# smearle/control-pcgrl

Hardware: AMD Instinct MI355X
Metric: env-steps/sec at N envs/GPU (binary 16x16), 1/2/4/8 MI355X (higher is better)
Workload: dtype u8

## Files before the change

### control_pcgrl_amd/_lib.py

```python
import ctypes as C
import os
import subprocess

_HERE = os.path.dirname(os.path.abspath(__file__))
CSRC = os.path.join(_HERE, "csrc")
LIB_PATH = os.path.join(CSRC, "libpcgrl_amd.so")
UNITS = ["pcgrl_engine.hip", "pcgrl_k_binary32.hip", "pcgrl_k_binary64.hip", "pcgrl_k_zelda32.hip", "pcgrl_k_zelda64.hip",
         "pcgrl_k_sokoban32_8.hip", "pcgrl_k_sokoban32_16.hip", "pcgrl_k_sokoban32_32.hip",
         "pcgrl_k_sokoban32_64.hip", "pcgrl_k_sokoban64_32.hip", "pcgrl_k_sokoban64_64.hip", "pcgrl_k_3d.hip",
         "codes/pcgrl_codes.hip", "reps3d/pcgrl_k_3d_turtle.hip", "reps3d/pcgrl_k_3d_wide.hip",
         "async3d/pcgrl_k_3d_async.hip", "paths/pcgrl_k_paths_binary.hip", "paths/pcgrl_k_paths_zelda.hip",
         "solutions/pcgrl_k_solutions.hip", "multiagent/pcgrl_k_ma_binary.hip", "multiagent/pcgrl_k_ma_zelda.hip",
         "measures/pcgrl_k_measures.hip", "smb/pcgrl_k_smb.hip", "smb/pcgrl_k_smb_env.hip", "smb/pcgrl_k_smb_ready.hip",
         "smb/pcgrl_k_smb_state.hip", "smb/pcgrl_k_smb_rollout.hip", "smb/pcgrl_k_smb_vector.hip",
         "smb/pcgrl_k_smb_measures.hip", "loderunner/pcgrl_k_loderunner.hip",
         "loderunner/pcgrl_k_loderunner_measures.hip", "loderunner/pcgrl_k_loderunner_routes.hip",
         "microstructure/pcgrl_k_microstructure.hip", "ddave/pcgrl_k_ddave.hip",
         "mdungeon/pcgrl_k_mdungeon.hip"]
HEADERS = ["pcgrl_kernels2d.h", "pcgrl_kernels3d.h", "pcgrl_sokoban.h", "pcgrl_common.h", "pcgrl_dispatch.h", "codes/pcgrl_codes.h",
           "reps3d/pcgrl_reps3d.h", "async3d/pcgrl_async3d.h", "paths/pcgrl_paths.h",
           "solutions/pcgrl_solutions.h", "multiagent/pcgrl_multiagent.h", "measures/pcgrl_measures.h",
           "smb/pcgrl_smb.h", "smb/pcgrl_smb_env.h", "smb/pcgrl_smb_ready.h", "smb/pcgrl_smb_state.h",
           "smb/pcgrl_smb_rollout.h", "smb/pcgrl_smb_ctrl.h", "smb/pcgrl_smb_vector.h", "smb/pcgrl_smb_measures.h",
           "loderunner/pcgrl_loderunner.h", "measures/pcgrl_measures_wave.h", "loderunner/pcgrl_loderunner_measures.h",
           "loderunner/pcgrl_loderunner_routes.h", "microstructure/pcgrl_microstructure.h", "ddave/pcgrl_ddave.h",
           "mdungeon/pcgrl_mdungeon.h"]
SOURCES = UNITS + HEADERS
HEADER = os.path.join(os.path.dirname(_HERE), "include", "pcgrl_amd.h")
CODES_HEADER = os.path.join(os.path.dirname(_HERE), "include", "pcgrl_amd_codes.h")
ASYNC3D_HEADER = os.path.join(os.path.dirname(_HERE), "include", "pcgrl_amd_async3d.h")
PATHS_HEADER = os.path.join(os.path.dirname(_HERE), "include", "pcgrl_amd_paths.h")
SOLUTIONS_HEADER = os.path.join(os.path.dirname(_HERE), "include", "pcgrl_amd_solutions.h")
MULTIAGENT_HEADER = os.path.join(os.path.dirname(_HERE), "include", "pcgrl_amd_multiagent.h")
MEASURES_HEADER = os.path.join(os.path.dirname(_HERE), "include", "pcgrl_amd_measures.h")
SMB_HEADER = os.path.join(os.path.dirname(_HERE), "include", "pcgrl_amd_smb.h")
SMB_ENV_HEADER = os.path.join(os.path.dirname(_HERE), "include", "pcgrl_amd_smb_env.h")
SMB_READY_HEADER = os.path.join(os.path.dirname(_HERE), "include", "pcgrl_amd_smb_ready.h")
SMB_STATE_HEADER = os.path.join(os.path.dirname(_HERE), "include", "pcgrl_amd_smb_state.h")
SMB_ROLLOUT_HEADER = os.path.join(os.path.dirname(_HERE), "include", "pcgrl_amd_smb_rollout.h")
SMB_CTRL_HEADER = os.path.join(os.path.dirname(_HERE), "include", "pcgrl_amd_smb_ctrl.h")
SMB_VECTOR_HEADER = os.path.join(os.path.dirname(_HERE), "include", "pcgrl_amd_smb_vector.h")
SMB_MEASURES_HEADER = os.path.join(os.path.dirname(_HERE), "include", "pcgrl_amd_smb_measures.h")
LODERUNNER_HEADER = os.path.join(os.path.dirname(_HERE), "include", "pcgrl_amd_loderunner.h")
LODERUNNER_MEASURES_HEADER = os.path.join(os.path.dirname(_HERE), "include", "pcgrl_amd_loderunner_measures.h")
LODERUNNER_ROUTES_HEADER = os.path.join(os.path.dirname(_HERE), "include", "pcgrl_amd_loderunner_routes.h")
MICROSTRUCTURE_HEADER = os.path.join(os.path.dirname(_HERE), "include", "pcgrl_amd_microstructure.h")
DDAVE_HEADER = os.path.join(os.path.dirname(_HERE), "include", "pcgrl_amd_ddave.h")
MDUNGEON_HEADER = os.path.join(os.path.dirname(_HERE), "include", "pcgrl_amd_mdungeon.h")
HIPCC_FLAGS = ["--offload-arch=gfx950", "-O3", "-std=c++17", "-ffp-contract=off", "-falign-loops=32", "-fPIC"]

PCGRL_MAX_STATS = 8
ERRORS = {1: "EINVAL", 2: "EUNSUPPORTED", 3: "EHIP", 4: "EACTION", 5: "ESTALE"}


class PcgrlConfig(C.Structure):
    _fields_ = [
        ("problem", C.c_int32), ("representation", C.c_int32), ("ndim", C.c_int32),
        ("dims", C.c_int32 * 3), ("obs_window", C.c_int32 * 3),
        ("max_iterations", C.c_int32), ("max_changes", C.c_int32), ("n_stats", C.c_int32),
        ("has_trg", C.c_int32 * PCGRL_MAX_STATS), ("weights", C.c_double * PCGRL_MAX_STATS),
        ("trg_lo", C.c_double * PCGRL_MAX_STATS), ("trg_hi", C.c_double * PCGRL_MAX_STATS),
        ("solver_power", C.c_int32),
        ("n_ctrl", C.c_int32), ("ctrl_idx", C.c_int32 * PCGRL_MAX_STATS), ("ctrl_range", C.c_double * PCGRL_MAX_STATS),
        ("act_window", C.c_int32 * 3), ("static_tiles", C.c_int32), ("n_static_walls", C.c_int32),
        ("static_eval", C.c_int32), ("static_prob", C.c_double),
    ]


SYMBOLS = {
    "pcgrl_create": (C.c_int, [C.POINTER(PcgrlConfig), C.c_int32, C.c_int32, C.POINTER(C.c_void_p)]),
    "pcgrl_destroy": (None, [C.c_void_p]),
    "pcgrl_seed": (C.c_int, [C.c_void_p, C.c_void_p]),
    "pcgrl_reset": (C.c_int, [C.c_void_p, C.c_void_p, C.c_void_p, C.c_void_p, C.c_void_p]),
    "pcgrl_step_seq": (C.c_int, [C.c_void_p, C.c_void_p, C.c_int64, C.c_int32, C.c_int32, C.c_int32, C.c_int32, C.c_void_p,
                                 C.c_void_p, C.c_void_p, C.c_void_p, C.c_void_p]),
    "pcgrl_step": (C.c_int, [C.c_void_p, C.c_void_p, C.c_int32, C.c_void_p, C.c_void_p, C.c_void_p, C.c_void_p,
                             C.c_void_p]),
    "pcgrl_step_ex": (C.c_int, [C.c_void_p, C.c_void_p, C.c_int32, C.c_void_p, C.c_void_p, C.c_void_p, C.c_void_p,
                                C.c_void_p, C.c_void_p, C.c_void_p]),
# ... 368 lines not shown
```

### control_pcgrl_amd/csrc/pcgrl_engine.hip

```cpp
#include <hip/hip_runtime.h>

#include <algorithm>
#include <cmath>
#include <cstddef>
#include <cstdio>
#include <cstring>
#include <string>
#include <vector>

#include <map>
#include <mutex>
#include <tuple>

#include "pcgrl_common.h"
#include "pcgrl_dispatch.h"
#include "pcgrl_kernels2d.h"
#include "pcgrl_sokoban.h"
#include "pcgrl_kernels3d.h"
#include "codes/pcgrl_codes.h"
#include "reps3d/pcgrl_reps3d.h"
#include "async3d/pcgrl_async3d.h"
#include "paths/pcgrl_paths.h"
#include "solutions/pcgrl_solutions.h"
#include "multiagent/pcgrl_multiagent.h"
#include "measures/pcgrl_measures.h"
#include "smb/pcgrl_smb.h"
#include "../../include/pcgrl_amd_codes.h"
#include "../../include/pcgrl_amd_async3d.h"
#include "../../include/pcgrl_amd_paths.h"
#include "../../include/pcgrl_amd_solutions.h"
#include "../../include/pcgrl_amd_multiagent.h"
#include "../../include/pcgrl_amd_measures.h"
#include "../../include/pcgrl_amd_smb.h"
#include "../../include/pcgrl_amd_smb_env.h"
#include "smb/pcgrl_smb_env.h"
#include "../../include/pcgrl_amd_smb_ready.h"
#include "smb/pcgrl_smb_ready.h"
#include "../../include/pcgrl_amd_smb_state.h"
#include "smb/pcgrl_smb_state.h"
#include "../../include/pcgrl_amd_smb_rollout.h"
#include "smb/pcgrl_smb_rollout.h"
#include "../../include/pcgrl_amd_smb_ctrl.h"
#include "smb/pcgrl_smb_ctrl.h"
#include "../../include/pcgrl_amd_smb_vector.h"
#include "smb/pcgrl_smb_vector.h"
#include "../../include/pcgrl_amd_smb_measures.h"
#include "smb/pcgrl_smb_measures.h"
#include "../../include/pcgrl_amd_loderunner.h"
#include "loderunner/pcgrl_loderunner.h"
#include "../../include/pcgrl_amd_loderunner_routes.h"
#include "loderunner/pcgrl_loderunner_routes.h"
#include "../../include/pcgrl_amd_loderunner_measures.h"
#include "loderunner/pcgrl_loderunner_measures.h"
#include "../../include/pcgrl_amd_microstructure.h"
#include "microstructure/pcgrl_microstructure.h"
#include "../../include/pcgrl_amd_ddave.h"
#include "ddave/pcgrl_ddave.h"
#include "../../include/pcgrl_amd_mdungeon.h"
#include "mdungeon/pcgrl_mdungeon.h"

using namespace pcgrl;

static thread_local std::string g_err;
static int fail(int code, const std::string &msg) {
  g_err = msg;
  return code;
}
#define HIPCHK(x)                                                                                   \
  do {                                                                                              \
    hipError_t _e = (x);                                                                            \
    if (_e != hipSuccess) return fail(PCGRL_EHIP, std::string(#x) + ": " + hipGetErrorString(_e)); \
  } while (0)

namespace pcgrl {
struct RedScratch;
struct SampleState;
}
struct pcgrl_engine {
  Params p;
  int device = 0;
  int lpe = 16;
  size_t lds_bytes = 0;
  int cpl = 0;
  int32_t *seen_host = nullptr;
  int soko_slots = 0;
  int32_t seen_last = 0, spread_left = 0;
  bool soko_lazy = true;
  int sk_budget = 0;
  void *a3_park = nullptr;
  void *sk_ws = nullptr, *sk_park = nullptr;
  bool soko_grow_failed = false;
  std::string soko_grow_msg;
  uint8_t *hdr_host = nullptr;
  int rollout_form = -1;
  int rollout_epw = -1;
  bool split_ok = false;
  int64_t two_role_resident = 0;
  hipStream_t side = nullptr;
  hipEvent_t ev_fork = nullptr, ev_join = nullptr;
  void *snap_planes = nullptr;
  EnvState *snap_st = nullptr;
  RngState *snap_rng = nullptr;
  long obs_nt_mb = 384;
  bool maybe_stale = false;
  int64_t obs_bytes = 0;
  int obs_ndim = 0;
  int32_t obs_shape[4] = {0, 0, 0, 0};
  RedScratch *red = nullptr;
  SampleState *sample = nullptr;
  bool ma_on = false;
  MaArgs ma = {};
  size_t ma_lds = 0;
  int64_t ma_obs_bytes = 0;
  int32_t ma_obs_shape[3] = {0, 0, 0};
  std::vector<void *> allocs;
  std::vector<std::pair<void *, size_t>> state_arrays;
};

extern "C" {
static void state_header_build(pcgrl_engine *h);
}

static void seedseq_words(uint64_t seed, uint64_t out[4]) {
  const uint32_t INIT_A = 0x43b0d7e5u, MULT_A = 0x931e8875u, INIT_B = 0x8b51f9ddu, MULT_B = 0x58f38dedu;
  const uint32_t MIX_L = 0xca01f9ddu, MIX_R = 0x4973f715u;
  uint32_t ent[4] = {(uint32_t)seed, (uint32_t)(seed >> 32), 0, 0};
  int n_ent = ent[1] ? 2 : 1;
  uint32_t pool[4], hc = INIT_A;
  auto hashmix = [&](uint32_t v) {
    v ^= hc;
    hc *= MULT_A;
    v *= hc;
    v ^= v >> 16;
    return v;
  };
  for (int i = 0; i < 4; i++) pool[i] = hashmix(i < n_ent ? ent[i] : 0u);
  for (int s = 0; s < 4; s++)
    for (int d = 0; d < 4; d++)
      if (s != d) {
        uint32_t r = MIX_L * pool[d] - MIX_R * hashmix(pool[s]);
        r ^= r >> 16;
        pool[d] = r;
      }
  uint32_t w[8], hb = INIT_B;
  for (int i = 0; i < 8; i++) {
    uint32_t v = pool[i & 3] ^ hb;
    hb *= MULT_B;
// ... 104 lines not shown
    return fail(PCGRL_EUNSUPPORTED, "sokoban: solver_power must be in [1, " + std::to_string(SK_MAX_POWER) +
                                        "] (the device solver's visited table and node ids are sized for that)");
  lpe = H <= 8 ? 8 : (H <= 16 ? 16 : (H <= 32 ? 32 : 64));
  if (W > 32 && lpe < 32) lpe = 32;
  if (c.representation == PCGRL_REP_WIDE) {
    if (c.obs_window[0] != H || c.obs_window[1] != W)
      return fail(PCGRL_EINVAL, "wide representation needs obs_window == map_shape (reference wrappers.py:140-150 reshape)");
    if (H != W) return fail(PCGRL_EUNSUPPORTED, "wide representation: the reference's transposed write needs a square map");
    obs_chunks = (W * nt + 15) / 16;
    obs_bytes = (int64_t)H * W * nt;
    shape[0] = H;
    shape[1] = W;
    shape[2] = nt;
    ndim = 3;
  } else {
    const int OH = c.obs_window[0], OW = c.obs_window[1], C = nt + 1 + (c.static_tiles ? 1 : 0);
    if (OH < 1 || OW < 1) return fail(PCGRL_EINVAL, "obs_window must be positive");
    obs_chunks = (OW * C + 15) / 16;
    obs_bytes = (int64_t)OH * OW * C;
    shape[0] = OH;
    shape[1] = OW;
    shape[2] = C;
    ndim = 3;
  }
  return PCGRL_OK;
}

static std::vector<JumpEntry> make_jump_table(int H, int W, int last = -1) {
  std::vector<JumpEntry> t(H + 1);
  U128 A{0, 1}, G{0, 0};
  const U128 a{PCG_MULT_HI, PCG_MULT_LO};
  int k = 0;
  for (int r = 0; r <= H; r++) {
    const int want = (r == H && last >= 0) ? last : r * W;
    if (want < k) {
      A = U128{0, 1};
      G = U128{0, 0};
      k = 0;
    }
    while (k < want) {
      G = add128(mul128(G, a), U128{0, 1});
      A = mul128(A, a);
      k++;
    }
    t[r] = JumpEntry{A.hi, A.lo, G.hi, G.lo};
  }
  return t;
}

static bool obs_nt_for(const pcgrl_engine *e, int64_t bytes_per_launch) {
  return e->obs_nt_mb > 0 && bytes_per_launch >= (int64_t)e->obs_nt_mb * 1000000;
}

static hipError_t launch(KernelId id, int lpe, const Params &p, size_t lds, hipStream_t s, int cpl = 0) {
  const bool wide64 = p.cfg.dims[1] > 32;
  switch (p.cfg.problem) {
    case PCGRL_PROB_MC3DMAZE:
      if (p.cfg.representation == PCGRL_REP_TURTLE) return launch_3d_turtle(id, p, cpl, s);
      if (p.cfg.representation == PCGRL_REP_WIDE) return launch_3d_wide(id, p, cpl, s);
      if (p.sk_budget > 0 && (id == K_STEP || id == K_RESET)) return launch_3d_async(id, p, cpl, s);
      return launch_3d(id, p, cpl, s);
    case PCGRL_PROB_BINARY: return wide64 ? launch_binary64(id, lpe, p, lds, s) : launch_binary32(id, lpe, p, lds, s);
    case PCGRL_PROB_ZELDA: return wide64 ? launch_zelda64(id, lpe, p, lds, s) : launch_zelda32(id, lpe, p, lds, s);
    default: return wide64 ? launch_sokoban64(id, lpe, p, lds, s) : launch_sokoban32(id, lpe, p, lds, s);
  }
}

struct DeviceGuard {
  int prev = -1;
  hipError_t err;
  explicit DeviceGuard(int device) {
    err = hipGetDevice(&prev);
    if (err == hipSuccess && prev != device) err = hipSetDevice(device);
    else if (err == hipSuccess) prev = -1;
  }
  ~DeviceGuard() {
    if (prev >= 0) (void)hipSetDevice(prev);
  }
};
#define ON_DEVICE(dev)                                                                            \
  DeviceGuard _guard(dev);                                                                        \
  if (_guard.err != hipSuccess) return fail(PCGRL_EHIP, std::string("hipSetDevice: ") + hipGetErrorString(_guard.err))

namespace pcgrl {

__global__ __launch_bounds__(64) void queue_targets_kernel(Params p, const double *lo, const double *hi) {
  const int env = blockIdx.x * 64 + threadIdx.x;
  if (env >= p.n_envs || (p.mask != nullptr && p.mask[env] == 0)) return;
  double *q = p.trg_pending + (size_t)env * PCGRL_MAX_STATS * 2;
  for (int k = 0; k < p.cfg.n_stats; k++) {
    q[2 * k] = lo[(size_t)env * p.cfg.n_stats + k];
    q[2 * k + 1] = hi[(size_t)env * p.cfg.n_stats + k];
  }
  p.trg_flag[env] |= 1;
}

constexpr int RED_BLOCKS = 64, RED_THREADS = 256, RED_W = 3 + PCGRL_MAX_STATS;
struct RedScratch {
  double part[RED_BLOCKS][RED_W];
  unsigned int ticket;
};
__global__ __launch_bounds__(RED_THREADS) void reduce_episodes_kernel(Params p, RedScratch *scr, double *out, int n_blocks, int clear) {
  __shared__ double sh[RED_THREADS / 64][RED_W];
  __shared__ bool last;
  const int chunk = (p.n_envs + n_blocks - 1) / n_blocks;
  const int lo = blockIdx.x * chunk, hi = min(p.n_envs, lo + chunk);
  double ret = 0.0;
  int64_t v[RED_W - 1];
// ... 193 lines not shown
  }
  (void)hipGetLastError();
  h->soko_grow_failed = true;
  h->soko_grow_msg = std::string("solver pool: growing from ") + std::to_string(h->soko_slots) + " to " + std::to_string(want) +
                     " slots failed: " + hipGetErrorString(e);
  return lazy ? PCGRL_OK : fail(PCGRL_EHIP, h->soko_grow_msg);
}

static void soko_pool_lazy(pcgrl_engine *h, Params &p, hipStream_t stream) {
  if (!h->seen_host || h->soko_slots >= sokoban_slots_for(h->p.n_envs)) return;
  if (*(volatile int32_t *)h->seen_host != 0) soko_pool_for(h, p, sokoban_slots_for(h->p.n_envs), stream);
}

static void choose_spread(pcgrl_engine *h, Params &p) {
  if (!h->seen_host || h->p.ext) return;
  static const int force = getenv("PCGRL_FORCE_SPREAD") ? atoi(getenv("PCGRL_FORCE_SPREAD")) : 0;
  if (force) {
    p.spread = 1;
    p.sk_helpers = force == 2 ? 3 : 0;
    return;
  }
  if (h->p.n_envs > 8192) return;
  const int32_t seen = *(volatile int32_t *)h->seen_host;
  if (seen != h->seen_last) {
    h->seen_last = seen;
    h->spread_left = 16;
  }
  if (h->spread_left > 0) {
    h->spread_left--;
    p.spread = 1;
    p.sk_helpers = h->lds_bytes + 3 * (size_t)SK_HELPER_LDS + 4096 <= 160 * 1024 ? 3 : 0;
  }
}

extern "C" {

const char *pcgrl_last_error(void) { return g_err.c_str(); }
const char *pcgrl_version(void) { return "pcgrl_amd 0.7.0 (gfx950)"; }

int pcgrl_create(const pcgrl_config *cfg, int32_t n_envs, int32_t device, pcgrl_handle *out) {
  if (!cfg || !out || n_envs < 1) return fail(PCGRL_EINVAL, "pcgrl_create: bad arguments");
  int lpe = 16, obs_chunks = 0, ndim = 0;
  int64_t obs_bytes = 0;
  int32_t shape[4] = {0, 0, 0, 0};
  int rc = validate(*cfg, lpe, obs_bytes, obs_chunks, shape, ndim);
  if (rc) return rc;
  ON_DEVICE(device);
  pcgrl_engine *e = new pcgrl_engine();
  {
    const char *f = getenv("PCGRL_ROLLOUT_KERNEL");
    if (f != nullptr && (f[0] == '0' || f[0] == '1')) e->rollout_form = f[0] - '0';
    if (getenv("PCGRL_OBS_NT_MB")) e->obs_nt_mb = atol(getenv("PCGRL_OBS_NT_MB"));
    if (getenv("PCGRL_ROLLOUT_EPW")) e->rollout_epw = atoi(getenv("PCGRL_ROLLOUT_EPW"));
  }
  e->device = device;
  e->lpe = lpe;
  e->obs_bytes = obs_bytes;
  e->obs_ndim = ndim;
  memcpy(e->obs_shape, shape, sizeof(shape));
  Params &p = e->p;
  memset(&p, 0, sizeof(p));
  p.cfg = *cfg;
  {
    bool integral = true;
    for (int k = 0; k < PCGRL_MAX_STATS; k++) {
      const double lo = cfg->trg_lo[k], hi = cfg->trg_hi[k];
      const int32_t big = 1 << 29;
      int32_t lo_i = 0, hi_i = 0;
      if (k < cfg->n_stats && cfg->has_trg[k]) {
        if (lo != lo || hi != hi || lo > hi) integral = false;
        else {
          if (lo <= -(double)big) lo_i = -big;
          else if (lo >= (double)big) lo_i = big;
          else if (lo == (double)(int32_t)lo) lo_i = (int32_t)lo;
          else integral = false;
          if (hi >= (double)big) hi_i = big;
          else if (hi <= -(double)big) hi_i = -big;
          else if (hi == (double)(int32_t)hi) hi_i = (int32_t)hi;
          else integral = false;
        }
      }
      p.trg_lo_i[k] = lo_i;
      p.trg_hi_i[k] = hi_i;
    }
    p.int_targets = integral ? 1 : 0;
  }
  p.n_envs = n_envs;
  p.n_tiles = n_tiles_of(cfg->problem);
  const bool is3d = cfg->problem == PCGRL_PROB_MC3DMAZE;
  p.n_cells = cfg->dims[0] * cfg->dims[1] * (is3d ? cfg->dims[2] : 1);
  p.obs_chunks = obs_chunks;
  if (is3d) m3_edge_masks_host(cfg->dims[1], cfg->dims[2], p.m3_notx0, p.m3_notxl);
  p.ext = (!is3d && (cfg->static_tiles || cfg->act_window[0] > 0)) ? 1 : 0;
  p.n_act = (!is3d && cfg->act_window[0] > 0) ? cfg->act_window[0] * cfg->act_window[1] : 1;
  e->lds_bytes = (size_t)(obs_chunks * 16 + 32) * (65 + (cfg->static_tiles ? 16 : 0)) + 64 * 8;
  {
    const int Hc = cfg->dims[0], Wc = cfg->dims[1], OWc = cfg->obs_window[1], Cc = p.n_tiles + 1;
    const bool fast_cfg = Hc == 16 && Wc == 16 && cfg->obs_window[0] == 32 && OWc == 32;
    p.obs16 = (!is3d && fast_cfg) ? 1 : 0;
    if ((p.obs16 || is3d) && obs_nt_for(e, (int64_t)n_envs * obs_bytes)) p.obs16 |= 2;
    if (!is3d && cfg->representation != PCGRL_REP_WIDE && !cfg->static_tiles && !fast_cfg && (OWc * Cc) % 16 == 0 &&
        e->lds_bytes > 20000) {
      const int rs = (Wc + 8 + 12 + 15) & ~15;
      const int epw = 64 / lpe;
      p.obs_codes = rs;
      e->lds_bytes = (size_t)epw * Hc * rs + rs + (size_t)Cc * 48 + 64 * 8;
// ... 144 lines not shown
  if (h->ma_on) HIPCHK(hipMemset2D(h->ma.side + 1, 4 * sizeof(uint32_t), 0, 2 * sizeof(uint32_t), (size_t)h->p.n_envs));
  return PCGRL_OK;
}

static void with_budget(const pcgrl_engine *h, Params &p) {
  p.sk_budget = h->sk_budget;
  if (h->sk_budget > 0 && h->a3_park) p.soko = h->a3_park;
}
static bool async_capable(const pcgrl_engine *h) {
  return h->p.soko != nullptr || (h->p.cfg.problem == PCGRL_PROB_MC3DMAZE && h->p.cfg.representation == PCGRL_REP_NARROW);
}

#define NOT_ATTACHED(h, what)                                                                                             \
  if ((h)->ma_on)                                                                                                         \
  return fail(PCGRL_EINVAL, std::string(what) + ": the engine steps several agents (pcgrl_ma_attach): use the pcgrl_ma_* entry " \
                                                "points of pcgrl_amd_multiagent.h")

int pcgrl_reset(pcgrl_handle h, const uint8_t *d_mask, const uint8_t *d_init_grids, const int32_t *d_init_pos, void *stream) {
  if (!h) return fail(PCGRL_EINVAL, "pcgrl_reset: null handle");
  NOT_ATTACHED(h, "pcgrl_reset");
  ON_DEVICE(h->device);
  Params p = h->p;
  soko_pool_lazy(h, p, (hipStream_t)stream);
  p.mask = d_mask;
  p.init_grids = d_init_grids;
  p.init_pos = d_init_pos;
  with_budget(h, p);
  HIPCHK(launch(K_RESET, h->lpe, p, h->lds_bytes, (hipStream_t)stream, h->cpl));
  if (d_mask == nullptr) h->maybe_stale = false;
  return PCGRL_OK;
}

#define NOT_WITH_BUDGET(h, what)                                                                                         \
  if ((h)->sk_budget > 0)                                                                                                \
  return fail(PCGRL_EINVAL, std::string(what) + ": a solver budget is set (pcgrl_set_solver_budget): envs may be busy, which only " \
                                                "pcgrl_step_ready can report")

int pcgrl_step(pcgrl_handle h, const int32_t *d_actions, int32_t auto_reset, uint8_t *d_obs, float *d_reward, uint8_t *d_done,
               int32_t *d_stats, void *stream) {
  if (!h || !d_actions) return fail(PCGRL_EINVAL, "pcgrl_step: bad arguments");
  NOT_WITH_BUDGET(h, "pcgrl_step");
  NOT_ATTACHED(h, "pcgrl_step");
  ON_DEVICE(h->device);
  Params p = h->p;
  p.no_fast = h->maybe_stale ? 1 : 0;
  soko_pool_lazy(h, p, (hipStream_t)stream);
  choose_spread(h, p);
  p.actions = d_actions;
  p.auto_reset = auto_reset;
  p.obs = d_obs;
  p.reward = d_reward;
  p.done = d_done;
  p.stats_out = d_stats;
  HIPCHK(launch(K_STEP, h->lpe, p, h->lds_bytes, (hipStream_t)stream, h->cpl));
  return PCGRL_OK;
}

int pcgrl_step_seq(pcgrl_handle h, const int32_t *d_action_rows, int64_t row_stride, int32_t n_rows, int32_t first_row,
                   int32_t n_steps, int32_t auto_reset, uint8_t *d_obs, float *d_reward, uint8_t *d_done, int32_t *d_stats,
                   void *stream) {
  if (!h || !d_action_rows || n_rows < 1 || n_steps < 0 || first_row < 0 || row_stride < 0)
    return fail(PCGRL_EINVAL, "pcgrl_step_seq: bad arguments");
  for (int32_t k = 0; k < n_steps; k++) {
    const int rc = pcgrl_step(h, d_action_rows + (size_t)((first_row + k) % n_rows) * (size_t)row_stride, auto_reset, d_obs, d_reward,
                              d_done, d_stats, stream);
    if (rc != PCGRL_OK) return rc;
  }
  return PCGRL_OK;
}

int pcgrl_step_ex(pcgrl_handle h, const int32_t *d_actions, int32_t auto_reset, uint8_t *d_obs, float *d_reward,
                  double *d_reward64, uint8_t *d_done, int32_t *d_stats, float *d_ctrl_obs, void *stream) {
  if (!h || !d_actions) return fail(PCGRL_EINVAL, "pcgrl_step_ex: bad arguments");
  NOT_WITH_BUDGET(h, "pcgrl_step_ex");
  NOT_ATTACHED(h, "pcgrl_step_ex");
  ON_DEVICE(h->device);
  if (d_ctrl_obs && h->p.cfg.n_ctrl == 0) return fail(PCGRL_EINVAL, "pcgrl_step_ex: d_ctrl_obs needs cfg.n_ctrl > 0");
  Params p = h->p;
  p.no_fast = h->maybe_stale ? 1 : 0;
  soko_pool_lazy(h, p, (hipStream_t)stream);
  choose_spread(h, p);
  p.actions = d_actions;
  p.auto_reset = auto_reset;
  p.obs = d_obs;
  p.reward = d_reward;
  p.reward64 = d_reward64;
  p.done = d_done;
  p.stats_out = d_stats;
  p.ctrl_obs = d_ctrl_obs;
  HIPCHK(launch(K_STEP, h->lpe, p, h->lds_bytes, (hipStream_t)stream, h->cpl));
  return PCGRL_OK;
}

static bool rollout_as_steps(const pcgrl_engine *h) {
  if (h->rollout_form >= 0) return h->rollout_form == 0;
  return h->p.cfg.problem != PCGRL_PROB_MC3DMAZE && (h->p.obs_codes > 0 || h->lpe > 16);
}

int32_t pcgrl_rollout_is_one_launch(pcgrl_handle h) { return h ? (rollout_as_steps(h) ? 0 : 1) : -1; }

int pcgrl_set_rollout_form(pcgrl_handle h, int32_t form) {
  if (!h || form < -1 || form > 2)
    return fail(PCGRL_EINVAL, "pcgrl_set_rollout_form: form must be -1 (by shape), 0 (step launches), 1 (one kernel) or 2 (two kernels)");
  if (form == 2 && !h->split_ok)
    return fail(PCGRL_EUNSUPPORTED, "pcgrl_set_rollout_form(2): the two-kernel rollout exists for 16 x 16 maps with the default window, plain mode");
  h->rollout_form = form;
  return PCGRL_OK;
}

int pcgrl_rollout_ex(pcgrl_handle h, const int32_t *d_actions, int32_t n_steps, int32_t auto_reset, uint8_t *d_obs,
                     int32_t obs_last_only, float *d_reward, double *d_reward64, uint8_t *d_done, int32_t *d_stats, float *d_ctrl_obs,
                     void *stream) {
  if (!h || !d_actions || n_steps < 1) return fail(PCGRL_EINVAL, "pcgrl_rollout: bad arguments");
  NOT_WITH_BUDGET(h, "pcgrl_rollout");
  NOT_ATTACHED(h, "pcgrl_rollout");
  if (d_ctrl_obs && h->p.cfg.n_ctrl == 0) return fail(PCGRL_EINVAL, "pcgrl_rollout_ex: d_ctrl_obs needs cfg.n_ctrl > 0");
  if (rollout_as_steps(h)) {
    const size_t N = (size_t)h->p.n_envs;
    for (int32_t k = 0; k < n_steps; k++) {
      const bool last = k == n_steps - 1;
      uint8_t *obs_k = d_obs == nullptr ? nullptr : (obs_last_only ? (last ? d_obs : nullptr) : d_obs + (size_t)k * N * (size_t)h->obs_bytes);
      const int rc = pcgrl_step_ex(h, d_actions + (size_t)k * N * (size_t)h->p.n_act, auto_reset, obs_k, d_reward ? d_reward + (size_t)k * N : nullptr,
                                   d_reward64 ? d_reward64 + (size_t)k * N : nullptr, d_done ? d_done + (size_t)k * N : nullptr,
                                   d_stats ? d_stats + (size_t)k * N * (size_t)h->p.cfg.n_stats : nullptr, last ? d_ctrl_obs : nullptr, stream);
      if (rc != PCGRL_OK) return rc;
    }
    return PCGRL_OK;
  }
  ON_DEVICE(h->device);
  Params p = h->p;
  p.no_fast = h->maybe_stale ? 1 : 0;
  soko_pool_lazy(h, p, (hipStream_t)stream);
  p.actions = d_actions;
  p.n_steps = n_steps;
  p.spread = 0;
  const bool roles_ok = h->split_ok && !h->maybe_stale && d_reward64 == nullptr && d_ctrl_obs == nullptr && h->rollout_form != 1;
  const int64_t two_role_wgs = ((int64_t)h->p.n_envs + 64 / h->lpe - 1) / (64 / h->lpe);
  const bool in_rounds = h->two_role_resident > 0 && two_role_wgs > h->two_role_resident;
  const bool split = roles_ok && d_obs != nullptr && (h->rollout_form == 2 || (in_rounds && !obs_last_only && n_steps >= 16));
  const bool sim_then_observe = roles_ok && !split && d_obs != nullptr && obs_last_only && in_rounds;
  const bool sim_only = (roles_ok && d_obs == nullptr) || sim_then_observe;
  if (h->p.cfg.problem != PCGRL_PROB_MC3DMAZE) {
    const int full = 64 / h->lpe;
// ... 15 lines not shown
    hipStream_t s0 = (hipStream_t)stream;
    if (split) {
      const int64_t plane_q = (int64_t)h->p.n_envs * ROW_WORDS * h->p.cfg.dims[0] * (int64_t)sizeof(uint32_t) / 16;
      const int64_t total = plane_q + (int64_t)h->p.n_envs * 2 + (int64_t)h->p.n_envs * (int64_t)(sizeof(RngState) / 16);
      hipLaunchKernelGGL(rollout_snapshot_kernel, dim3((unsigned)((total + 255) / 256)), dim3(256), 0, s0, (const uint4 *)h->p.planes,
                         (uint4 *)h->snap_planes, plane_q, (const uint4 *)h->p.st, (uint4 *)h->snap_st, (const uint4 *)h->p.rng, (uint4 *)h->snap_rng,
                         h->p.n_envs);
      HIPCHK(hipGetLastError());
      HIPCHK(hipEventRecord(h->ev_fork, s0));
      HIPCHK(hipStreamWaitEvent(h->side, h->ev_fork, 0));
      Params po = p;
      po.planes = h->snap_planes;
      po.st = h->snap_st;
      po.rng = h->snap_rng;
      po.spread = 0;
      po.reward = nullptr;
      po.done = nullptr;
      po.stats_out = nullptr;
      HIPCHK(launch(K_ROLLOUT_OBS, h->lpe, po, h->lds_bytes, h->side, h->cpl));
    }
    Params ps = p;
    ps.obs = nullptr;
    HIPCHK(launch(K_ROLLOUT_SIM, h->lpe, ps, 0, s0, h->cpl));
    if (split) {
      HIPCHK(hipEventRecord(h->ev_join, h->side));
      HIPCHK(hipStreamWaitEvent(s0, h->ev_join, 0));
    }
    if (sim_then_observe) {
      Params po = h->p;
      po.obs = d_obs;
      HIPCHK(launch(K_OBSERVE, h->lpe, po, h->lds_bytes, s0, h->cpl));
    }
    return PCGRL_OK;
  }
  HIPCHK(launch(K_ROLLOUT, h->lpe, p, h->lds_bytes, (hipStream_t)stream, h->cpl));
  return PCGRL_OK;
}

int pcgrl_rollout(pcgrl_handle h, const int32_t *d_actions, int32_t n_steps, int32_t auto_reset, uint8_t *d_obs,
                  int32_t obs_last_only, float *d_reward, uint8_t *d_done, int32_t *d_stats, void *stream) {
  return pcgrl_rollout_ex(h, d_actions, n_steps, auto_reset, d_obs, obs_last_only, d_reward, nullptr, d_done, d_stats, nullptr, stream);
}

int pcgrl_update(pcgrl_handle h, const int32_t *d_actions, uint8_t *d_obs, void *stream) {
  if (!h || !d_actions) return fail(PCGRL_EINVAL, "pcgrl_update: bad arguments");
  NOT_WITH_BUDGET(h, "pcgrl_update");
  NOT_ATTACHED(h, "pcgrl_update");
  ON_DEVICE(h->device);
  Params p = h->p;
  p.actions = d_actions;
  p.obs = d_obs;
  p.update_only = 1;
  h->maybe_stale = true;
  HIPCHK(launch(K_STEP, h->lpe, p, h->lds_bytes, (hipStream_t)stream, h->cpl));
  return PCGRL_OK;
}

int pcgrl_refresh_stats(pcgrl_handle h, int32_t *d_stats, void *stream) {
  if (!h) return fail(PCGRL_EINVAL, "pcgrl_refresh_stats: null handle");
  ON_DEVICE(h->device);
  Params p = h->p;
  p.refresh_only = 1;
  p.stats_out = d_stats;
  with_budget(h, p);
  HIPCHK(launch(K_RESET, h->lpe, p, h->lds_bytes, (hipStream_t)stream, h->cpl));
  h->maybe_stale = false;
  return PCGRL_OK;
}

int pcgrl_queue_targets(pcgrl_handle h, const uint8_t *d_mask, const double *d_trg_lo, const double *d_trg_hi, void *stream) {
  if (!h || !d_trg_lo || !d_trg_hi) return fail(PCGRL_EINVAL, "pcgrl_queue_targets: bad arguments");
  ON_DEVICE(h->device);
  if (h->p.cfg.n_ctrl == 0) return fail(PCGRL_EINVAL, "pcgrl_queue_targets: the engine was created without control metrics");
  Params p = h->p;
  p.mask = d_mask;
  hipLaunchKernelGGL(queue_targets_kernel, dim3((p.n_envs + 63) / 64), dim3(64), 0, (hipStream_t)stream, p, d_trg_lo, d_trg_hi);
  HIPCHK(hipGetLastError());
  return PCGRL_OK;
}

int pcgrl_set_target_resampling(pcgrl_handle h, int32_t enable, uint64_t seed, const double *lo, const double *hi) {
  if (!h) return fail(PCGRL_EINVAL, "pcgrl_set_target_resampling: null handle");
  if (h->p.cfg.n_ctrl == 0) return fail(PCGRL_EINVAL, "pcgrl_set_target_resampling: the engine was created without control metrics");
  if (enable && (!lo || !hi)) return fail(PCGRL_EINVAL, "pcgrl_set_target_resampling: bounds missing");
  ON_DEVICE(h->device);
  TrgResample r;
  memset(&r, 0, sizeof(r));
  r.enable = enable ? 1 : 0;
  r.seed = seed;
  for (int j = 0; j < h->p.cfg.n_ctrl && enable; j++) {
    if (!(lo[j] <= hi[j])) return fail(PCGRL_EINVAL, "pcgrl_set_target_resampling: need lo <= hi for every control metric");
    r.lo[j] = lo[j];
    r.hi[j] = hi[j];
  }
  HIPCHK(hipDeviceSynchronize());
  HIPCHK(hipMemcpy((TrgResample *)h->p.trg - 1, &r, sizeof(r), hipMemcpyHostToDevice));
  return PCGRL_OK;
}

int pcgrl_ctrl_observe(pcgrl_handle h, float *d_ctrl_obs, void *stream) {
  if (!h || !d_ctrl_obs) return fail(PCGRL_EINVAL, "pcgrl_ctrl_observe: bad arguments");
  ON_DEVICE(h->device);
  if (h->p.cfg.n_ctrl == 0) return fail(PCGRL_EINVAL, "pcgrl_ctrl_observe: the engine was created without control metrics");
  Params p = h->p;
  p.ctrl_obs = d_ctrl_obs;
  dim3 grid((p.n_envs + 63) / 64), block(64);
  switch (p.cfg.n_stats) {
// ... 375 lines not shown
    if (e != hipSuccess) {
      (void)hipGetLastError();
      return fail(PCGRL_EHIP, std::string("pcgrl_set_solver_budget: allocating one park record per env: ") + hipGetErrorString(e));
    }
    h->a3_park = pool;
  }
  if (!maze3d && budget > 0 && h->sk_ws == nullptr) {
    HIPCHK(hipDeviceSynchronize());
    const hipError_t e = sokoban_alloc_async(h->p, h->allocs, h->p.n_envs, &h->sk_ws, &h->sk_park);
    if (e != hipSuccess) {
      (void)hipGetLastError();
      return fail(PCGRL_EHIP, std::string("pcgrl_set_solver_budget: allocating one solver workspace per env: ") + hipGetErrorString(e));
    }
  }
  if (budget == 0 && h->sk_budget > 0) {
    HIPCHK(hipDeviceSynchronize());
    std::vector<EnvState> st(h->p.n_envs);
    HIPCHK(hipMemcpy(st.data(), h->p.st, st.size() * sizeof(EnvState), hipMemcpyDeviceToHost));
    for (auto &e : st)
      if (e.flags & (ENV_PENDING_STEP | ENV_PENDING_STATS))
        return fail(PCGRL_EINVAL, "pcgrl_set_solver_budget(0): an env is still busy (a parked search): keep stepping with pcgrl_step_ready "
                                  "or reset the envs first");
  }
  h->sk_budget = budget;
  return PCGRL_OK;
}

int32_t pcgrl_get_solver_budget(pcgrl_handle h) { return h ? h->sk_budget : -1; }

int64_t pcgrl_park_bytes_per_env(pcgrl_handle h) {
  if (!h) return -1;
  if (h->p.cfg.problem != PCGRL_PROB_MC3DMAZE || h->p.cfg.representation != PCGRL_REP_NARROW) return 0;
  return (int64_t)a3_park_bytes(h->p.cfg.dims[0], h->p.cfg.dims[1], h->p.cfg.dims[2]);
}

int pcgrl_step_ready(pcgrl_handle h, const int32_t *d_actions, int32_t auto_reset, uint8_t *d_obs, float *d_reward, uint8_t *d_done,
                     int32_t *d_stats, uint8_t *d_status, void *stream) {
  if (!h || !d_actions || !d_status) return fail(PCGRL_EINVAL, "pcgrl_step_ready: bad arguments");
  if (h->sk_budget <= 0) return fail(PCGRL_EINVAL, "pcgrl_step_ready: no solver budget set (pcgrl_set_solver_budget)");
  ON_DEVICE(h->device);
  Params p = h->p;
  p.no_fast = h->maybe_stale ? 1 : 0;
  soko_pool_lazy(h, p, (hipStream_t)stream);
  p.spread = 1;
  p.sk_helpers = 0;
  with_budget(h, p);
  p.actions = d_actions;
  p.auto_reset = auto_reset;
  p.obs = d_obs;
  p.reward = d_reward;
  p.done = d_done;
  p.stats_out = d_stats;
  p.ready = d_status;
  HIPCHK(launch(K_STEP, h->lpe, p, h->lds_bytes, (hipStream_t)stream, h->cpl));
  return PCGRL_OK;
}

int pcgrl_env_busy(pcgrl_handle h, uint8_t *d_busy, void *stream) {
  if (!h || !d_busy) return fail(PCGRL_EINVAL, "pcgrl_env_busy: bad arguments");
  ON_DEVICE(h->device);
  hipLaunchKernelGGL(env_busy_kernel, dim3((h->p.n_envs + 255) / 256), dim3(256), 0, (hipStream_t)stream, h->p, d_busy);
  HIPCHK(hipGetLastError());
  return PCGRL_OK;
}

int pcgrl_reserve_solver_pool(pcgrl_handle h, int32_t n_slots, int32_t allow_lazy_growth) {
  if (!h) return fail(PCGRL_EINVAL, "pcgrl_reserve_solver_pool: null handle");
  if (!h->p.soko) return fail(PCGRL_EINVAL, "pcgrl_reserve_solver_pool: the engine has no device solver (sokoban only)");
  ON_DEVICE(h->device);
  h->soko_lazy = allow_lazy_growth != 0;
  const int full = sokoban_slots_for(h->p.n_envs);
  const int want = n_slots < 0 ? h->soko_slots : (n_slots == 0 ? full : std::min((int)n_slots, 512));
  Params scratch = h->p;
  return soko_pool_for(h, scratch, want, nullptr, false);
}

int32_t pcgrl_solver_pool_slots(pcgrl_handle h, int32_t *full_size_out, int32_t *grow_failed_out) {
  if (!h || !h->p.soko) return 0;
  if (full_size_out) *full_size_out = sokoban_slots_for(h->p.n_envs);
  if (grow_failed_out) *grow_failed_out = h->soko_grow_failed ? 1 : 0;
  if (h->soko_grow_failed) g_err = h->soko_grow_msg;
  return h->soko_slots;
}

int pcgrl_copy_to_host(void *dst_host, const void *d_src, int64_t bytes, void *stream) {
  if (!dst_host || !d_src || bytes < 0) return fail(PCGRL_EINVAL, "pcgrl_copy_to_host: bad arguments");
  HIPCHK(hipMemcpyAsync(dst_host, d_src, (size_t)bytes, hipMemcpyDeviceToHost, (hipStream_t)stream));
  return PCGRL_OK;
}

int pcgrl_stream_synchronize(void *stream) {
  HIPCHK(hipStreamSynchronize((hipStream_t)stream));
  return PCGRL_OK;
}

int pcgrl_graph_upload(void *graph_exec, void *stream) {
  if (!graph_exec) return fail(PCGRL_EINVAL, "pcgrl_graph_upload: null graph");
  HIPCHK(hipGraphUpload((hipGraphExec_t)graph_exec, (hipStream_t)stream));
  return PCGRL_OK;
}

int pcgrl_debug_counters(pcgrl_handle h, uint64_t *out, int32_t n) {
  if (!h || !out || n < 1 || n > 8 * (h->p.n_envs + 64)) return fail(PCGRL_EINVAL, "pcgrl_debug_counters: bad arguments");
  HIPCHK(hipSetDevice(h->device));
  HIPCHK(hipDeviceSynchronize());
  HIPCHK(hipMemcpy(out, h->p.err + 64, sizeof(uint64_t) * n, hipMemcpyDeviceToHost));
  HIPCHK(hipMemset(h->p.err + 64, 0, sizeof(uint64_t) * n));
// ... 1667 lines not shown
```

Before: 631.8 million.

## Add specialized step kernel for binary 16x16 with DPP-based BFS sweep

Adds a dedicated step kernel for binary 16x16 maps with narrow or turtle representation. Each block pairs an observer wave, which encodes observations and precomputes the flood component, with a stats wave. The BFS sweep expands six frontier levels per trip using inline DPP and bitop3 assembly, and the hot EnvState line is read and written as 16-byte words. The new kernel is on by default and can be switched off with PCGRL_STEP16=0, at the cost of hand-written gfx950-specific asm and duplicated step logic.

New measurement: 686.2 million (median of 6 runs). +8.6%, better.

```diff
diff --git a/control_pcgrl_amd/_lib.py b/control_pcgrl_amd/_lib.py
--- a/control_pcgrl_amd/_lib.py
+++ b/control_pcgrl_amd/_lib.py
@@ -16,7 +16,7 @@
          "smb/pcgrl_k_smb_measures.hip", "loderunner/pcgrl_k_loderunner.hip",
          "loderunner/pcgrl_k_loderunner_measures.hip", "loderunner/pcgrl_k_loderunner_routes.hip",
          "microstructure/pcgrl_k_microstructure.hip", "ddave/pcgrl_k_ddave.hip",
-         "mdungeon/pcgrl_k_mdungeon.hip"]
+         "mdungeon/pcgrl_k_mdungeon.hip", "step16/pcgrl_k_step16.hip"]
 HEADERS = ["pcgrl_kernels2d.h", "pcgrl_kernels3d.h", "pcgrl_sokoban.h", "pcgrl_common.h", "pcgrl_dispatch.h", "codes/pcgrl_codes.h",
            "reps3d/pcgrl_reps3d.h", "async3d/pcgrl_async3d.h", "paths/pcgrl_paths.h",
            "solutions/pcgrl_solutions.h", "multiagent/pcgrl_multiagent.h", "measures/pcgrl_measures.h",
@@ -24,7 +24,7 @@
            "smb/pcgrl_smb_rollout.h", "smb/pcgrl_smb_ctrl.h", "smb/pcgrl_smb_vector.h", "smb/pcgrl_smb_measures.h",
            "loderunner/pcgrl_loderunner.h", "measures/pcgrl_measures_wave.h", "loderunner/pcgrl_loderunner_measures.h",
            "loderunner/pcgrl_loderunner_routes.h", "microstructure/pcgrl_microstructure.h", "ddave/pcgrl_ddave.h",
-           "mdungeon/pcgrl_mdungeon.h"]
+           "mdungeon/pcgrl_mdungeon.h", "step16/pcgrl_step16.h"]
 SOURCES = UNITS + HEADERS
 HEADER = os.path.join(os.path.dirname(_HERE), "include", "pcgrl_amd.h")
 CODES_HEADER = os.path.join(os.path.dirname(_HERE), "include", "pcgrl_amd_codes.h")
diff --git a/control_pcgrl_amd/csrc/pcgrl_engine.hip b/control_pcgrl_amd/csrc/pcgrl_engine.hip
--- a/control_pcgrl_amd/csrc/pcgrl_engine.hip
+++ b/control_pcgrl_amd/csrc/pcgrl_engine.hip
@@ -58,6 +58,7 @@
 #include "ddave/pcgrl_ddave.h"
 #include "../../include/pcgrl_amd_mdungeon.h"
 #include "mdungeon/pcgrl_mdungeon.h"
+#include "step16/pcgrl_step16.h"
 
 using namespace pcgrl;
 
@@ -93,6 +94,7 @@
   std::string soko_grow_msg;
   uint8_t *hdr_host = nullptr;
   int rollout_form = -1;
+  bool step16 = true;
   int rollout_epw = -1;
   bool split_ok = false;
   int64_t two_role_resident = 0;
@@ -303,8 +305,9 @@
   return e->obs_nt_mb > 0 && bytes_per_launch >= (int64_t)e->obs_nt_mb * 1000000;
 }
 
-static hipError_t launch(KernelId id, int lpe, const Params &p, size_t lds, hipStream_t s, int cpl = 0) {
+static hipError_t launch(KernelId id, int lpe, const Params &p, size_t lds, hipStream_t s, int cpl = 0, bool step16 = false) {
   const bool wide64 = p.cfg.dims[1] > 32;
+  if (id == K_STEP && step16 && step16_applies(p, lpe)) return launch_step16(p, lds, s);
   switch (p.cfg.problem) {
     case PCGRL_PROB_MC3DMAZE:
       if (p.cfg.representation == PCGRL_REP_TURTLE) return launch_3d_turtle(id, p, cpl, s);
@@ -604,6 +607,8 @@
     if (f != nullptr && (f[0] == '0' || f[0] == '1')) e->rollout_form = f[0] - '0';
     if (getenv("PCGRL_OBS_NT_MB")) e->obs_nt_mb = atol(getenv("PCGRL_OBS_NT_MB"));
     if (getenv("PCGRL_ROLLOUT_EPW")) e->rollout_epw = atoi(getenv("PCGRL_ROLLOUT_EPW"));
+    const char *s16 = getenv("PCGRL_STEP16");
+    if (s16 != nullptr && s16[0] == '0') e->step16 = false;
   }
   e->device = device;
   e->lpe = lpe;
@@ -854,7 +859,7 @@
   p.reward = d_reward;
   p.done = d_done;
   p.stats_out = d_stats;
-  HIPCHK(launch(K_STEP, h->lpe, p, h->lds_bytes, (hipStream_t)stream, h->cpl));
+  HIPCHK(launch(K_STEP, h->lpe, p, h->lds_bytes, (hipStream_t)stream, h->cpl, h->step16));
   return PCGRL_OK;
 }
 
@@ -890,7 +895,7 @@
   p.done = d_done;
   p.stats_out = d_stats;
   p.ctrl_obs = d_ctrl_obs;
-  HIPCHK(launch(K_STEP, h->lpe, p, h->lds_bytes, (hipStream_t)stream, h->cpl));
+  HIPCHK(launch(K_STEP, h->lpe, p, h->lds_bytes, (hipStream_t)stream, h->cpl, h->step16));
   return PCGRL_OK;
 }
 
@@ -1012,7 +1017,7 @@
   p.obs = d_obs;
   p.update_only = 1;
   h->maybe_stale = true;
-  HIPCHK(launch(K_STEP, h->lpe, p, h->lds_bytes, (hipStream_t)stream, h->cpl));
+  HIPCHK(launch(K_STEP, h->lpe, p, h->lds_bytes, (hipStream_t)stream, h->cpl, h->step16));
   return PCGRL_OK;
 }
 
@@ -1494,7 +1499,7 @@
   p.done = d_done;
   p.stats_out = d_stats;
   p.ready = d_status;
-  HIPCHK(launch(K_STEP, h->lpe, p, h->lds_bytes, (hipStream_t)stream, h->cpl));
+  HIPCHK(launch(K_STEP, h->lpe, p, h->lds_bytes, (hipStream_t)stream, h->cpl, h->step16));
   return PCGRL_OK;
 }
 
diff --git a/control_pcgrl_amd/csrc/step16/pcgrl_k_step16.hip b/control_pcgrl_amd/csrc/step16/pcgrl_k_step16.hip
--- /dev/null
+++ b/control_pcgrl_amd/csrc/step16/pcgrl_k_step16.hip
@@ -0,0 +1,285 @@
+#include "pcgrl_step16.h"
+
+#include "../pcgrl_kernels2d.h"
+
+namespace pcgrl {
+
+#if defined(PCGRL_PHASE_TIMING) || defined(PCGRL_WAVE_TRACE)
+constexpr int STEP16_PAIRS = 1;
+#else
+constexpr int STEP16_PAIRS = 2;
+#endif
+
+typedef uint4 __attribute__((may_alias)) uint4_rec;
+typedef uint2 __attribute__((may_alias)) uint2_rec;
+
+#define STEP16_LEVEL(in, out)                                                              \
+  "v_lshlrev_b32 %6, 1, " in "\n\t"                                                        \
+  "v_lshrrev_b32 %7, 1, " in "\n\t"                                                        \
+  "v_or_b32_dpp %6, " in ", %6 row_shr:1 row_mask:0xf bank_mask:0xf bound_ctrl:1\n\t"      \
+  "v_or_b32_dpp %7, " in ", %7 row_shl:1 row_mask:0xf bank_mask:0xf bound_ctrl:1\n\t"      \
+  "v_bitop3_b32 " out ", %6, %7, %8 bitop3:0xa8\n\t"                                       \
+  "v_bitop3_b32 %8, %6, %7, %8 bitop3:2\n\t"
+__device__ __attribute__((always_inline)) inline void trip16(uint32_t f0, uint32_t &f1, uint32_t &f2, uint32_t &f3, uint32_t &f4,
+                                                             uint32_t &f5, uint32_t &f6, uint32_t &fr) {
+  uint32_t a, b;
+  asm(STEP16_LEVEL("%9", "%0") STEP16_LEVEL("%0", "%1") STEP16_LEVEL("%1", "%2") STEP16_LEVEL("%2", "%3")
+          STEP16_LEVEL("%3", "%4") STEP16_LEVEL("%4", "%5")
+      : "=&v"(f1), "=&v"(f2), "=&v"(f3), "=&v"(f4), "=&v"(f5), "=&v"(f6), "=&v"(a), "=&v"(b), "+v"(fr)
+      : "v"(f0));
+}
+#undef STEP16_LEVEL
+
+__device__ __attribute__((always_inline)) inline void sweep16(const Grp<16> &g, uint32_t src, uint32_t avail, int &len,
+                                                              uint32_t &last, uint32_t &visited) {
+  static_assert(SWEEP_UNROLL == 6, "sweep16 keeps six frontiers per trip");
+  constexpr uint64_t LOW = 0x7FFF7FFF7FFF7FFFull, TOP = 0x8000800080008000ull;
+  uint32_t front = src & avail;
+  uint32_t free_cells = avail & ~front;
+  uint32_t k0 = 0, k1 = 0, k2 = 0, k3 = 0, k4 = 0, k5 = 0;
+  int base = 0, lev = 0;
+  uint64_t alive = TOP;
+  while (true) {
+    const uint32_t f0 = front;
+    uint32_t f1, f2, f3, f4, f5;
+    trip16(f0, f1, f2, f3, f4, f5, front, free_cells);
+    const uint64_t bal = __ballot(front != 0);
+    const uint64_t now = (((bal & LOW) + LOW) | bal) & TOP;
+    const uint64_t gone = alive & ~now;
+    if (gone != 0) {
+      const bool died = ((gone >> (g.gbase + 15)) & 1ull) != 0;
+      k0 = died ? f0 : k0;
+      k1 = died ? f1 : k1;
+      k2 = died ? f2 : k2;
+      k3 = died ? f3 : k3;
+      k4 = died ? f4 : k4;
+      k5 = died ? f5 : k5;
+      base = died ? lev : base;
+    }
+    lev += SWEEP_UNROLL;
+    alive = now;
+    if (now == 0) break;
+  }
+  int myidx = k1 ? 1 : 0;
+  myidx = k2 ? 2 : myidx;
+  myidx = k3 ? 3 : myidx;
+  myidx = k4 ? 4 : myidx;
+  myidx = k5 ? 5 : myidx;
+  const int gidx = (int)g.gmax((uint32_t)myidx);
+  len = base + gidx;
+  uint32_t l = k0;
+  l = gidx == 1 ? k1 : l;
+  l = gidx == 2 ? k2 : l;
+  l = gidx == 3 ? k3 : l;
+  l = gidx == 4 ? k4 : l;
+  l = gidx == 5 ? k5 : l;
+  last = len > 0 ? l : 0u;
+  visited = avail & ~free_cells;
+}
+
+__device__ inline uint32_t component_fars16(const Grp<16> &g, uint32_t comps) {
+  const uint32_t iso = comps & ~expand(g, comps);
+  uint32_t remaining = comps & ~iso, fars = iso;
+  while (true) {
+    const uint64_t gb = g.gballot(remaining != 0);
+    if (__ballot(gb != 0) == 0) break;
+    const int fl = gb ? __builtin_ctzll(gb) : -1;
+    const uint32_t seed = g.row == fl ? (remaining & (0u - remaining)) : 0u;
+    int depth;
+    uint32_t last, vis;
+    sweep16(g, seed, remaining, depth, last, vis);
+    fars |= first_rowmajor(g, last);
+    remaining &= ~vis;
+  }
+  return fars;
+}
+
+__device__ inline void binary_stats_update16(const Grp<16> &g, uint32_t x, uint32_t p_old, uint32_t p_new, int &regions,
+                                             int &path_len, uint32_t &fars, uint32_t &best PHASE_ARG, bool have_pre, uint32_t pre) {
+  const bool became_pass = g.gany((x & p_new) != 0);
+  const bool edited = g.gany(x != 0);
+  uint32_t K = edited ? pre : 0u;
+  if (__ballot(edited && !have_pre) != 0) {
+    const uint32_t Kf = flood(g, x, became_pass ? p_new : p_old);
+    K = have_pre ? K : Kf;
+  }
+  K = became_pass ? K : (K & ~x);
+  const uint32_t touched = K | x;
+  const bool hit = g.gany((best & touched) != 0);
+  PHASE_MARK(3);
+  const uint32_t newfars = component_fars16(g, K);
+  PHASE_MARK(4);
+  fars = (fars & ~touched) | newfars;
+  int l;
+  uint32_t b, vis;
+  sweep16(g, hit ? fars : newfars, p_new, l, b, vis);
+  PHASE_MARK(5);
+  if (edited) {
+    regions = (int)g.gsum((uint32_t)popc_m(fars));
+    if (hit || l > path_len) {
+      path_len = l;
+      best = b;
+    }
+  } else {
+    (void)g.gsum(0u);
+  }
+}
+
+__global__ __launch_bounds__(128 * STEP16_PAIRS, PCGRL_STEP_WAVES) void step16_kernel(Params p) {
+  constexpr int PROB = PCGRL_PROB_BINARY, LPE = 16, NS = 2, EPW = 4;
+  typedef uint32_t M;
+  extern __shared__ __attribute__((aligned(16))) uint8_t lds_all[];
+  touch_kernarg(p);
+  Grp<LPE> g;
+  g.init();
+  const int wave = __builtin_amdgcn_readfirstlane((int)(threadIdx.x >> 6));
+  const int pair = wave >> 1;
+  const bool observer = (wave & 1) != 0;
+  uint8_t *lds = lds_all + (size_t)pair * p.lds_pair_bytes;
+  const int env = (int)((blockIdx.x * STEP16_PAIRS + pair) * EPW + (g.lane / LPE));
+  const bool active = env < p.n_envs;
+  const M colmask = active ? 0xFFFFu : 0u;
+  const int e = active ? env : 0;
+  M *pl = (M *)p.planes + (size_t)e * ROW_WORDS * 16 + g.row;
+  EnvState *S = &p.st[e];
+  uint64_t *rng_stash = (uint64_t *)(lds + p.lds_pair_bytes - 64 * EPW) + 8 * (g.lane / LPE);
+
+  if (observer) {
+    TRACE_DECL();
+    M b[1];
+    b[0] = active ? pl[0] : M(0);
+    const uint4 s0 = *(const uint4_rec *)S;
+    const uint2 s1 = *(const uint2_rec *)&S->iteration;
+    const int action = active ? p.actions[e] : 0;
+    if (p.auto_reset != 0 && g.row < 8) rng_stash[g.row] = ((const uint64_t *)&p.rng[e])[g.row];
+    __syncthreads();
+    int pos[2] = {(int)s0.x, (int)s0.y};
+    int n_step = (int)s0.w, iteration = (int)s1.x + 1, changes = (int)s1.y;
+    bool bad = false;
+    const bool change = rep_update<PROB, LPE, M, true>(g, p, active, action, b, pos, n_step, bad);
+    changes += change ? 1 : 0;
+    bool done = iteration > p.cfg.max_iterations;
+    if (p.cfg.max_changes >= 0) done = done || changes > p.cfg.max_changes;
+    const bool do_reset = active && done && p.auto_reset != 0;
+    if (__ballot(do_reset) != 0) {
+      Pcg obs_rp, obs_rr;
+      obs_rr.load(rng_stash);
+      obs_rp.load(rng_stash + 4);
+      reset_from_rng<PROB, LPE, M>(g, p, e, do_reset, b, pos, false, nullptr, &obs_rp, &obs_rr);
+    }
+    encode_obs_any<PROB, LPE, true, M>(g, p, e, active, b, pos, lds);
+    const M xbit = (active && g.row == pos[0]) ? (M(1) << pos[1]) : M(0);
+    const M comp = flood(g, xbit, (~b[0] & colmask) | xbit);
+    if (active) pl[16 * PRE_PLANE] = comp | (M)PRE_VALID;
+    TRACE_PUT(2, _tr0);
+    TRACE_PUT(3, TRACE_NOW());
+    TRACE_DRAIN();
+    TRACE_PUT(4, TRACE_NOW());
+    return;
+  }
+
+  if (p.n_envs <= 8192) __builtin_amdgcn_s_setprio(3);
+  PHASE_DECL();
+  TRACE_DECL();
+  M b[3];
+  b[0] = active ? pl[0] : M(0);
+  b[1] = active ? pl[16] : M(0);
+  b[2] = active ? pl[32] : M(0);
+  const M pre3 = active ? pl[16 * PRE_PLANE] : M(0);
+  const uint4 s0 = ((const uint4_rec *)S)[0];
+  const uint4 s1 = ((const uint4_rec *)S)[1];
+  const uint4 s2 = ((const uint4_rec *)S)[2];
+  const uint2 s4 = *(const uint2_rec *)&S->stats[0];
+  const int action = active ? p.actions[e] : 0;
+  static_assert(offsetof(EnvState, n_step) == 12 && offsetof(EnvState, iteration) == 16 && offsetof(EnvState, last_ep_len) == 28 &&
+                    offsetof(EnvState, last_loss) == 32 && offsetof(EnvState, ep_return) == 40 && offsetof(EnvState, stats) == 64,
+                "step16_kernel reads and writes the hot line of EnvState as 16-byte words");
+  __syncthreads();
+  PHASE_MARK(0);
+  int pos[2] = {(int)s0.x, (int)s0.y};
+  const uint32_t pos2 = s0.z;
+  int n_step = (int)s0.w, iteration = (int)s1.x + 1, changes = (int)s1.y, flags = (int)s1.z;
+  uint32_t last_ep_len = s1.w;
+  double last_loss = __hiloint2double((int)s2.y, (int)s2.x), ep_return = __hiloint2double((int)s2.w, (int)s2.z);
+  int32_t st[NS] = {(int32_t)s4.x, (int32_t)s4.y};
+  const M tile0_old = b[0];
+
+  bool bad = false;
+  const bool change = rep_update<PROB, LPE, M, true>(g, p, active, action, b, pos, n_step, bad);
+  changes += change ? 1 : 0;
+  bool done = iteration > p.cfg.max_iterations;
+  if (p.cfg.max_changes >= 0) done = done || changes > p.cfg.max_changes;
+  const bool do_reset = active && done && p.auto_reset != 0;
+  if (bad && g.row == 0 && active) atomicOr(p.err, 1);
+  PHASE_MARK(1);
+  if ((flags & ENV_STATS_DIRTY) != 0 && change && active && g.row == 0) atomicOr(p.err, 8);
+  if (__ballot(change) != 0) {
+    const M x = change ? (tile0_old ^ b[0]) & colmask : M(0);
+    int reg = st[0], len = st[1];
+    M fars = b[1], best = b[2];
+    binary_stats_update16(g, x, ~tile0_old & colmask, ~b[0] & colmask, reg, len, fars, best PHASE_PASS,
+                          g.gany((pre3 & (M)PRE_VALID) != 0), pre3 & colmask);
+    if (change) {
+      st[0] = reg;
+      st[1] = len;
+      b[1] = fars;
+      b[2] = best;
+    }
+  }
+  PHASE_MARK(2);
+  const double loss = get_loss<NS>(p, st);
+  const double rew = loss - last_loss;
+  last_loss = loss;
+  ep_return += rew;
+  if (active && g.row == 0) {
+    if (p.reward) p.reward[e] = (float)rew;
+    if (p.done) p.done[e] = done ? 1 : 0;
+    if (p.stats_out) {
+      p.stats_out[(size_t)e * NS] = st[0];
+      p.stats_out[(size_t)e * NS + 1] = st[1];
+    }
+  }
+  if (__ballot(do_reset) != 0) {
+    if (do_reset) last_ep_len = (uint32_t)iteration;
+    if (do_reset && g.row == 0) latch_episode<NS>(p, e, S, ep_return, iteration, st);
+    reset_from_rng<PROB, LPE, M>(g, p, e, do_reset, b, pos, true, nullptr);
+    int32_t ns[NS];
+    compute_stats<PROB, LPE, M, false>(g, p, e, do_reset, b, colmask, ns);
+    if (do_reset) {
+      st[0] = ns[0];
+      st[1] = ns[1];
+      iteration = 0;
+      changes = 0;
+      n_step = 0;
+      flags = 0;
+      ep_return = 0.0;
+      last_loss = get_loss<NS>(p, st);
+    }
+  }
+  if ((change || do_reset) && active) {
+    pl[0] = b[0];
+    pl[16] = b[1];
+    pl[32] = b[2];
+  }
+  if (active && g.row == 0) {
+    ((uint4_rec *)S)[0] = make_uint4((uint32_t)pos[0], (uint32_t)pos[1], pos2, (uint32_t)n_step);
+    ((uint4_rec *)S)[1] = make_uint4((uint32_t)iteration, (uint32_t)changes, (uint32_t)flags, last_ep_len);
+    ((uint4_rec *)S)[2] = make_uint4((uint32_t)__double2loint(last_loss), (uint32_t)__double2hiint(last_loss),
+                                     (uint32_t)__double2loint(ep_return), (uint32_t)__double2hiint(ep_return));
+    *(uint2_rec *)&S->stats[0] = make_uint2((uint32_t)st[0], (uint32_t)st[1]);
+    if (do_reset) accumulate_episode<NS>(S);
+  }
+  PHASE_MARK(6);
+  PHASE_FLUSH();
+  TRACE_PUT(0, _tr0);
+  TRACE_PUT(1, TRACE_NOW());
+}
+
+hipError_t launch_step16(const Params &p, size_t lds, hipStream_t s) {
+  const unsigned pairs = (unsigned)((p.n_envs + 3) / 4);
+  const dim3 grid((pairs + STEP16_PAIRS - 1) / STEP16_PAIRS);
+  hipLaunchKernelGGL(step16_kernel, grid, dim3(128 * STEP16_PAIRS), STEP16_PAIRS * lds, s, p);
+  return hipGetLastError();
+}
+
+}
diff --git a/control_pcgrl_amd/csrc/step16/pcgrl_step16.h b/control_pcgrl_amd/csrc/step16/pcgrl_step16.h
--- /dev/null
+++ b/control_pcgrl_amd/csrc/step16/pcgrl_step16.h
@@ -0,0 +1,19 @@
+#pragma once
+#include <hip/hip_runtime.h>
+
+#include "../pcgrl_common.h"
+
+namespace pcgrl {
+
+inline bool step16_applies(const Params &p, int lpe) {
+  const pcgrl_config &c = p.cfg;
+  const bool plain = p.trg == nullptr && p.reward64 == nullptr;
+  return c.problem == PCGRL_PROB_BINARY && lpe == 16 && c.dims[0] == 16 && c.dims[1] == 16 &&
+         (c.representation == PCGRL_REP_NARROW || c.representation == PCGRL_REP_TURTLE) && c.obs_window[0] == 32 &&
+         c.obs_window[1] == 32 && p.obs != nullptr && !p.no_fast && !p.update_only && !p.ext && c.n_ctrl == 0 && !p.spread &&
+         !p.sk_budget && !p.obs_codes && plain;
+}
+
+hipError_t launch_step16(const Params &p, size_t lds, hipStream_t s);
+
+}
```
